# JANUS-Institute/HallThrusterPEM

Measured on AMD Instinct MI355X. Metric: coupled PEM-v0 model evals/sec, higher is better.
Workload: dtype f64

## Files before the change

hallthrusterpem_amd/_lib.py:

```python
import ctypes as C
import importlib.util
import os
import threading
from pathlib import Path

PKG = Path(__file__).resolve().parent
LIB_PATH = PKG / 'libpem_hip.so'

PEM_OK, PEM_ERR_INVALID_ARG, PEM_ERR_HIP, PEM_ERR_NO_DEVICE = 0, 1, 2, 3
NANGLE = 91
FUSED_LATENT_MAX_RANK = 8
FUSED_SYSTEM_MAX_RECORDS = 1024
FUSED_SYSTEM_MAX_RADII = 8
SYS_JION, SYS_VCC, SYS_T, SYS_UION = 0, 1, 2, 3
SWEEP_CATHODE, SWEEP_THRUSTER, SWEEP_PLUME = 0, 1, 2
DE_MAX_POP, DE_MAX_DIM = 1024, 16
DE_BEST1BIN, DE_RAND1BIN = 0, 1
NM_MAX_DIM, NM_STATE_WORDS = 32, 10
POWELL_MAX_DIM, POWELL_STATE_WORDS = 32, 24
POWELL_SCALARS, POWELL_VEC_ROWS = 20, 6
DRAM_MAX_DIM = 32
ENSEMBLE_MAX_DIM, ENSEMBLE_MAX_WALKERS = 32, 1024
SMC_MAX_DIM, SMC_MAX_PARTICLES, SMC_BISECTIONS = 32, 16384, 52
CHAIN_TIME_BLOCK = 4096
# ... 70 lines not shown
    'pem_range_narrow_dev': (C.c_int, [C.c_int, C.c_int, _dp, _dp, _dp, _dp, _dp]),
    'pem_qsel_bins': (C.c_int, [C.c_int, C.c_int, C.POINTER(C.c_int), C.POINTER(C.c_int)]),
    'pem_qsel_minmax_f64_dev': (C.c_int, [_sz, C.c_int, _dp, _sz, _dp, _dp, _dp, _dp]),
    'pem_qsel_hist1_f64_dev': (C.c_int, [_sz, C.c_int, _dp, _sz, _dp, _dp, C.c_int, _dp, _dp]),
    'pem_qsel_decide1_dev': (C.c_int, [C.c_int, C.c_int, _dp, _dp, _dp, C.c_int, _dp, _dp, _dp, _dp, _dp]),
    'pem_qsel_hist2_f64_dev': (C.c_int, [_sz, C.c_int, _dp, _sz, _dp, _dp, C.c_int, _dp, C.c_int, C.c_int, _dp, _dp]),
    'pem_qsel_decide2_dev': (C.c_int, [C.c_int, C.c_int, _dp, _dp, C.c_int, _dp, _dp, _dp, _dp, _dp, _dp, _dp]),
    'pem_qsel_compact_f64_dev': (C.c_int, [_sz, C.c_int, _dp, _sz, _dp, _dp, C.c_int, _dp, _dp, _dp, C.c_int, C.c_int, C.c_uint32, _dp, _dp, _dp]),
    'pem_qsel_select_dev': (C.c_int, [C.c_int, C.c_int, C.c_int, C.c_uint32, _dp, _dp, _dp, _dp, _dp, _dp, _dp]),
    'pem_quantiles_f64_dev': (C.c_int, [_sz, C.c_int, _dp, _sz, C.c_int, _dp, _dp, _dp, _dp, _dp]),
    'pem_quantiles_strided_f64_dev': (C.c_int, [_sz, C.c_int, _dp, _sz, _sz, C.c_int, _dp, _dp, _dp, _dp, _dp]),
    'pem_quantiles_last_path': (C.c_int, []),
    'pem_coupled_mc_stats_f64_dev': (C.c_int, [_sz, C.c_uint64, C.c_uint64, C.c_uint32, _dp, _dp, _dp, C.c_double, C.c_double, _dp, _sz,
                                               _dp, _dp, _dp, _dp, _dp, _dp, _dp, _dp, C.c_int, _dp, _dp, _dp, _dp, _dp, _dp,
                                               C.c_int, C.c_int, C.c_double, _dp, _dp, _dp, _dp]),
    'pem_row_masks_f64_dev': (C.c_int, [_sz, C.c_int, _dp, _sz, _dp, _dp, _dp, _dp, _dp]),
    'pem_campaign_masks_f64_dev': (C.c_int, [_sz, C.c_int, _dp, _dp, C.c_int, C.c_int, C.c_int, C.c_double, _dp, _dp, _sz, _dp, _dp, C.c_int, _dp, _dp,
                                             C.c_int, _dp]),
    'pem_sobol_partial_f64_dev': (C.c_int, [_sz, C.c_int, _sz, _dp, _dp, _dp, _dp, C.c_int, _dp]),
    'pem_coupled_f32_dev': (C.c_int, [_sz, C.c_float, C.c_float, _dp, _sz, _dp, _sz, _dp, _dp]),
    'pem_saltelli_f32_dev': (C.c_int, [_sz, C.c_uint64, C.c_uint64, C.c_uint32, _dp, _dp, _dp, C.c_int, _dp, C.c_float, C.c_float, _dp, _dp, C.c_int, _dp]),
    'pem_saltelli_f64_dev': (C.c_int, [_sz, C.c_uint64, C.c_uint64, C.c_uint32, _dp, _dp, _dp, C.c_int, _dp, C.c_double, C.c_double, _dp, _dp, C.c_int, _dp]),
    'pem_saltelli_qmc_f32_dev': (C.c_int, [_sz, C.c_uint64, C.c_uint64, C.c_uint32, C.c_int, _dp, _dp, _dp, C.c_int, _dp, C.c_float, C.c_float, _dp, _dp,
                                           C.c_int, _dp]),
    'pem_saltelli_qmc_f64_dev': (C.c_int, [_sz, C.c_uint64, C.c_uint64, C.c_uint32, C.c_int, _dp, _dp, _dp, C.c_int, _dp, C.c_double, C.c_double, _dp,
                                           _dp, C.c_int, _dp]),
    'pem_saltelli2_f32_dev': (C.c_int, [_sz, C.c_uint64, C.c_uint64, C.c_uint32, _dp, _dp, _dp, C.c_int, _dp, _dp, C.c_float, C.c_float, _dp, _dp,
                                        C.c_int, _dp]),
    'pem_saltelli2_f64_dev': (C.c_int, [_sz, C.c_uint64, C.c_uint64, C.c_uint32, _dp, _dp, _dp, C.c_int, _dp, _dp, C.c_double, C.c_double, _dp, _dp,
                                        C.c_int, _dp]),
# ... 130 lines not shown
```

hallthrusterpem_amd/build.py:

```python
import os
import shutil
import subprocess
from pathlib import Path

PKG = Path(__file__).resolve().parent
ROOT = PKG.parent
SRCS = [PKG / 'csrc' / 'pem_kernels.hip', PKG / 'csrc' / 'pem_radii.hip', PKG / 'csrc' / 'pem_stages.hip', PKG / 'csrc' / 'pem_host.hip', PKG / 'csrc' / 'pem_campaign.hip', PKG / 'csrc' / 'pem_sampler.hip', PKG / 'csrc' / 'pem_svd.hip', PKG / 'csrc' / 'pem_likelihood.hip', PKG / 'csrc' / 'pem_surrogate.hip', PKG / 'csrc' / 'pem_surrogate_fields.hip', PKG / 'csrc' / 'pem_surrogate_sobol.hip', PKG / 'csrc' / 'pem_fp32.hip', PKG / 'csrc' / 'pem_saltelli.hip', PKG / 'csrc' / 'pem_saltelli2.hip', PKG / 'csrc' / 'pem_latent.hip', PKG / 'csrc' / 'pem_quantile.hip', PKG / 'csrc' / 'pem_masks.hip', PKG / 'csrc' / 'pem_sobol_sweep.hip', PKG / 'csrc' / 'pem_de.hip', PKG / 'csrc' / 'pem_nm.hip', PKG / 'csrc' / 'pem_powell.hip', PKG / 'csrc' / 'pem_dram.hip', PKG / 'csrc' / 'pem_ensemble.hip', PKG / 'csrc' / 'pem_tempering.hip', PKG / 'csrc' / 'pem_smc.hip', PKG / 'csrc' / 'pem_chains.hip', PKG / 'csrc' / 'pem_marginals.hip', PKG / 'csrc' / 'pem_hexbin.hip', PKG / 'csrc' / 'pem_information.hip', PKG / 'csrc' / 'pem_qmc.hip']
LIB = PKG / 'libpem_hip.so'
DEPS = SRCS + sorted((PKG / 'csrc').glob('*.h')) + [ROOT / 'include' / 'pem_hip.h']


def hipcc() -> str:
    exe = shutil.which('hipcc') or '/opt/rocm/bin/hipcc'
    if not Path(exe).exists():
        raise RuntimeError('hipcc not found: libpem_hip.so cannot be built (ROCm toolchain required)')
    return exe


def have_hipcc() -> bool:
    return Path(shutil.which('hipcc') or '/opt/rocm/bin/hipcc').exists()


STAMP = PKG / 'libpem_hip.so.srchash'

# ... 76 lines not shown
```

hallthrusterpem_amd/csrc/pem_qfused.h:

```cpp
#pragma once
#include <hip/hip_runtime.h>

#include <cstdint>

namespace pem {

struct Bracket {
    unsigned long long lo, hi;
    unsigned loh;
    unsigned words;
    unsigned mult;
    unsigned pad;
};

struct Record {
    unsigned long long key;
    unsigned long long col;
};

__device__ __forceinline__ unsigned long long order_key(double x) {
    const unsigned long long b = (unsigned long long)__double_as_longlong(x);
    return (b >> 63) ? ~b : (b | 0x8000000000000000ull);
}
__device__ __forceinline__ unsigned order_key_high(int high_word) {
// ... 24 lines not shown
    size_t ld = 0;
    double *V_cc = nullptr, *I_B0 = nullptr, *T = nullptr, *j_ion = nullptr, *div_angle = nullptr, *T_c = nullptr;
    uint8_t* invalid = nullptr;
};

__attribute__((visibility("hidden"))) int launch_coupled_mc(const McLaunch& a, hipStream_t st);
__attribute__((visibility("hidden"))) int coupled_count_waves(size_t n, int nq, bool store_profile, unsigned* waves);
__attribute__((visibility("hidden"))) int launch_coupled_mc_count(const McLaunch& a, const CountIO& c, bool store_profile, hipStream_t st);

struct FusedProducer {
    virtual ~FusedProducer() {}
    int pm_q25 = -1, pm_q75 = -1;
    double pm_factor = 0.0;
    uint8_t *pm_certain = nullptr, *pm_uncertain = nullptr;
    int pm_done = 0;
    virtual int pilot(size_t rows, double* dst, hipStream_t st) = 0;
    virtual int waves(int nq, unsigned* waves) = 0;
    virtual int count(const CountIO& io, hipStream_t st) = 0;
};
__attribute__((visibility("hidden"))) int quantiles_fused(size_t n, int m, int nq, const uint64_t* rank_prev, const uint64_t* rank_next,
                                                          const double* gamma, double* pilot_rows, FusedProducer& prod, double* out,
                                                          int* fused_ok, hipStream_t st);
struct SidePlan {
    int (*before_full)(void* ctx, hipStream_t st) = nullptr;
    void* ctx = nullptr;
};
__attribute__((visibility("hidden"))) int quantiles_side(size_t n, int m, const double* data, size_t ld, size_t cs, int nq,
                                                         const uint64_t* rank_prev, const uint64_t* rank_next, const double* gamma, double* out,
                                                         hipStream_t st, const SidePlan* plan = nullptr);

// ... 2 lines not shown
```

hallthrusterpem_amd/csrc/pem_quantile.hip:

```cpp
#include <hip/hip_runtime.h>

#include <atomic>
#include <cmath>
#include <cstdint>
#include <cstdlib>
#include <mutex>

#include "pem_common.h"
#include "pem_hip.h"
#include "pem_qfused.h"

namespace {

typedef unsigned long long u64;
constexpr int QBLOCK = 512;
constexpr int QWAVES = QBLOCK / 64;
constexpr int LDS_WORDS = 36864;
constexpr int SORT_CAP = 4096;
constexpr int SORT_DIRECT = 512;
constexpr int MAX_NC = 4;
constexpr int UNROLL = 8;
static_assert(PEM_QUANTILE_MAX_Q == 6, "hist2_kernel / compact_kernel are instantiated for 2, 4, ... 12 ranks per column");

__device__ __forceinline__ u64 key_of(double x) {
// ... 1176 lines not shown
        if (const char* e = getenv("PEM_FUSED_PILOT")) pilot = atoll(e) >= 32 ? atoll(e) : 32;
    }
    if (plan) pilot = 32;
    const bool use_pilot = fused ? true : plan ? (long long)n >= 4 * pilot : (pilot >= 2 && (long long)n * m >= pilot_min && (long long)n >= 4 * pilot);
    if (fused && (long long)n < 4 * pilot) return pem::fail(PEM_ERR_INVALID_ARG, "pem_quantiles: the fused form needs at least %lld rows", 4 * pilot);

    const size_t b_col = sizeof(Column) * m, b_tg = sizeof(Target) * m * nt;
    const size_t b_h1 = sizeof(unsigned) * (size_t)m * bins1, b_h2 = sizeof(unsigned) * (size_t)m * nt * bins2;
    const size_t b_br = sizeof(Bracket) * m * nq, b_bl = sizeof(u64) * m * nq, b_hA = sizeof(unsigned) * (size_t)m * nq * binsA;
    auto up = [](size_t x) { return (x + 255) & ~(size_t)255; };
    const size_t o_tg = up(b_col), o_h1 = o_tg + up(b_tg), o_h2 = o_h1 + up(b_h1), o_tot = o_h2 + up(b_h2);
    unsigned fused_waves = 0;
    if (fused)
        if (int rc = fused->waves(nq, &fused_waves)) return rc;
    const size_t b_rc = sizeof(unsigned) * fused_waves;
    const size_t o_br = o_tot + 256, o_bl = o_br + up(b_br), o_hA = o_bl + up(b_bl), o_rc = o_hA + up(b_hA), o_pm = o_rc + up(b_rc);
    const size_t o_end = o_pm + up(sizeof(uint4) * (size_t)m);
    QWork& work = g_qwork[slot];
    std::lock_guard<std::mutex> lock(work.mu);
    char*& ws_buf = work.ws_buf;
    size_t &ws_cap = work.ws_cap, &cand_cap = work.cand_cap, &rec_cap = work.rec_cap, &part_cap = work.part_cap;
    u64*& cand_buf = work.cand_buf;
    pem::Record*& rec_buf = work.rec_buf;
    unsigned*& part_buf = work.part_buf;
    int& ws_dev = work.ws_dev;
    int dev = 0;
    HIP_TRY(hipGetDevice(&dev));
    if (dev != ws_dev || ws_cap < o_end) {
        if (ws_buf) (void)hipFree(ws_buf);
        if (cand_buf && dev != ws_dev) {
            (void)hipFree(cand_buf);
// ... 18 lines not shown
    }
    char* ws = ws_buf;
    Column* col = reinterpret_cast<Column*>(ws);
    Target* tg = reinterpret_cast<Target*>(ws + o_tg);
    unsigned* hist1 = reinterpret_cast<unsigned*>(ws + o_h1);
    unsigned* hist2 = reinterpret_cast<unsigned*>(ws + o_h2);
    u64* total = reinterpret_cast<u64*>(ws + o_tot);
    int* outside = reinterpret_cast<int*>(total + 1);
    int* incomplete = reinterpret_cast<int*>(total + 2);
    int* any_single = reinterpret_cast<int*>(total + 8);
    int* unfit = reinterpret_cast<int*>(total + 9);
    int* prod_flags = unfit + 1;
    unsigned* rec_count = reinterpret_cast<unsigned*>(ws + o_rc);
    uint4* pm_thr = reinterpret_cast<uint4*>(ws + o_pm);
    int* pm_bad = unfit + 3;
    int* inconsistent = unfit + 4;
    Bracket* br = reinterpret_cast<Bracket*>(ws + o_br);
    u64* below = reinterpret_cast<u64*>(ws + o_bl);
    unsigned* histA = reinterpret_cast<unsigned*>(ws + o_hA);
    auto cleanup = [&](int code) {
        (void)hipStreamSynchronize(st);
        return code;
    };
#define Q_TRY(expr)                                                                                          \
    do {                                                                                                     \
        hipError_t e_ = (expr);                                                                              \
        if (e_ != hipSuccess) return cleanup(pem::fail(PEM_ERR_HIP, "%s: %s", #expr, hipGetErrorString(e_))); \
    } while (0)

    Wanted w{};
    for (int q = 0; q < nq; ++q) {
        w.prev[q] = rank_prev[q];
        w.next[q] = rank_next[q];
        w.gamma[q] = gamma[q];
    }
    const int cblocks = (m + 63) / 64;
    const int nc = m <= 64 ? 1 : (m <= 128 ? 2 : 4);
    const size_t lds1 = (size_t)m * bins1 * 4, lds2 = (size_t)m * nt * bins2 * 4, ldsA = (size_t)m * nq * (binsA + 1) * 4;
    const dim3 blk(QBLOCK);
    auto grid_for = [&](size_t rows) {
        const long long rpw = m <= 64 ? 64 / m : 1, groups = ((long long)rows + rpw - 1) / rpw;
        long long blocks = (groups + (long long)QWAVES * UNROLL - 1) / ((long long)QWAVES * UNROLL);
        if (blocks > 256 * 2) blocks = 256 * 2;
        return dim3((unsigned)blocks);
// ... 101 lines not shown
        PilotEnds ends{};
        const double n1 = n > 1 ? (double)(n - 1) : 1.0, np1 = (double)(rows_p - 1);
        for (int q = 0; q < nq; ++q) {
            const double p_lo = (double)rank_prev[q] / n1, p_hi = (double)rank_next[q] / n1;
            double sig = fused ? 5.0 : 7.0;
            if (fused)
                if (const char* e = getenv("PEM_FUSED_SIGMA")) sig = atof(e) >= 3.0 ? atof(e) : 3.0;
            const double d_lo = sig * sqrt((double)rows_p * p_lo * (1.0 - p_lo)) + 8.0, d_hi = sig * sqrt((double)rows_p * p_hi * (1.0 - p_hi)) + 8.0;
            const double r_lo = floor(p_lo * np1 - d_lo) - 1.0, r_hi = ceil(p_hi * np1 + d_hi) + 1.0;
            ends.open_lo[q] = r_lo < 0.0;
            ends.open_hi[q] = r_hi > np1;
            pw.prev[q] = ends.open_lo[q] ? 0 : (u64)r_lo;
            pw.next[q] = ends.open_hi[q] ? (u64)(rows_p - 1) : (u64)r_hi;
        }
        if (fused) {
            if (int rc = fused->pilot(rows_p, const_cast<double*>(data), st)) return cleanup(rc);
            const bool edges = !(getenv("PEM_FUSED_PILOT_EXACT") && atoi(getenv("PEM_FUSED_PILOT_EXACT")));
            if (int rc = four_passes(rows_p, ld, pw, edges)) return rc;
        } else if (plan) {
            if (int rc = four_passes(rows_p, ld, pw)) return rc;
            if (plan->before_full)
                if (int rc = plan->before_full(plan->ctx, st)) return cleanup(rc);
        } else if (int rc = four_passes(rows_p, ld * (size_t)pilot, pw)) return rc;
        const dim3 grid = grid_for(n);
        Q_TRY(hipMemsetAsync(total, 0, 256, st));
        Q_TRY(hipMemsetAsync(below, 0, o_end - o_bl, st));
        hipLaunchKernelGGL(brackets_kernel, dim3((unsigned)((m * nq + 63) / 64)), dim3(64), 0, st, m, nq, tg, ends, binsA, br, any_single);
        hipLaunchKernelGGL(init_columns_kernel, dim3(cblocks), dim3(64), 0, st, col, tg, m, nq, w);
#define Q_BRHIST_(NC_, NQ_)                                                                                                  \
    Q_LDS((bracket_hist_kernel<NC_, NQ_>));                                                                                  \
    hipLaunchKernelGGL((bracket_hist_kernel<NC_, NQ_>), grid, blk, ldsA, st, (long long)n, m, ld, cs, data, br, any_single, binsA, col, below, histA)
#define Q_BRHIST(NC_) Q_BY_NQ_##NC_(Q_BRHIST_, NC_)
        unsigned rcap = 0;
// ... 69 lines not shown
            hipLaunchKernelGGL(record_reduce_kernel, dim3((unsigned)((cells + 63) / 64)), dim3(256), 0, st, part_buf, cus, cells, histA, rec_count, rcap,
                               fused_waves, rec_sums);
            hipLaunchKernelGGL(record_total_check_kernel, dim3(1), dim3(64), 0, st, rec_sums, inconsistent, prod_flags);
        }
        hipLaunchKernelGGL(decide_bracket_kernel, dim3((unsigned)(m * nt)), dim3(64), 0, st, nt, col, br, below, histA, binsA, tg, outside);
        hipLaunchKernelGGL(layout_kernel, dim3(1), dim3(64 * MAX_NC), 0, st, m, nt, tg, total);
        Q_TRY(hipGetLastError());
        u64 h_tot[2] = {0, 0};
        int h_unfit4[4] = {0, 0, 0, 0};
        Q_TRY(hipMemcpyAsync(h_tot, total, 2 * sizeof(u64), hipMemcpyDeviceToHost, st));
        if (fused) Q_TRY(hipMemcpyAsync(h_unfit4, unfit, sizeof h_unfit4, hipMemcpyDeviceToHost, st));
        Q_TRY(hipStreamSynchronize(st));
        if (fused) fused->pm_done = (pm_launched && h_unfit4[3] == 0) ? 1 : 0;
        if (fused && (h_unfit4[0] || (int)(h_tot[1] & 0xffffffffull) != 0 || h_unfit4[1] || h_unfit4[2])) {
            *fused_ok = 0;
            return cleanup(PEM_OK);
        }
        if ((int)(h_tot[1] & 0xffffffffull) == 0) {
            Q_TRY(grow_candidates(h_tot[0]));
            u64* cand = cand_buf;
#define Q_BRCOMPACT_(NC_, NQ_) \
    hipLaunchKernelGGL((compact_bracket_kernel<NC_, NQ_>), grid, blk, 0, st, (long long)n, m, ld, cs, data, br, tg, cand)
#define Q_BRCOMPACT(NC_) Q_BY_NQ_##NC_(Q_BRCOMPACT_, NC_)
            if (!fused) {
                Q_BY_NC(Q_BRCOMPACT);
            } else {
                int cus = 256;
                Q_TRY(pem::device_cus(&cus));
                unsigned* woff = part_buf + (size_t)cus * m * nq * binsA;
                hipLaunchKernelGGL(record_offsets_kernel, dim3((unsigned)(m * nt)), dim3(64), 0, st, nt, binsA, tg, part_buf, cus, m * nq * binsA, woff);
// ... 626 lines not shown
```

hallthrusterpem_amd/drivers.py:

```python
import functools

import numpy as np

from . import sampling
from .batch import QOI_NAMES, CoupledBatch
from .distributed import shard_bounds

COORDS_STR_ID = '_coords'


MAX_Q, MAX_Q_WIDE = 6, 3


def _linear_ranks(n: int, percentiles):
    return _linear_ranks_cached(int(n), tuple(float(x) for x in np.atleast_1d(np.asarray(percentiles, dtype=np.float64))))


@functools.lru_cache(maxsize=64)
def _linear_ranks_cached(n: int, percentiles: tuple):
    q = np.true_divide(np.asarray(percentiles, dtype=np.float64), np.float64(100))
    if not np.all((q >= 0) & (q <= 1)):
        raise ValueError('Percentiles must be in the range [0, 100]')
    if n == 0:
        raise ValueError('no samples')
# ... 176 lines not shown
            for k in names if k in outputs}


def _stacked_rows(tensors):
    import torch
    t0 = tensors[0]
    if len(tensors) < 2 or any(t.dim() != 1 or not t.is_cuda or t.dtype != torch.float64 or t.numel() != t0.numel() or t.stride(0) != 1
                               or t.untyped_storage().data_ptr() != t0.untyped_storage().data_ptr() for t in tensors):
        return None
    n, step = t0.numel(), tensors[1].storage_offset() - t0.storage_offset()
    if step < n or any(t.storage_offset() != t0.storage_offset() + i * step for i, t in enumerate(tensors)):
        return None
    return torch.as_strided(t0, (n, len(tensors)), (1, step))


def campaign_statistics(outputs: dict, iqr_factor: float = 1.5, percentiles=(5.0, 50.0, 95.0), names=None):
    import torch
    names = [k for k in (outputs if names is None else names) if k in outputs and COORDS_STR_ID not in str(k) and str(k) != 'errors']
    pct = [25.0, 75.0] + [float(x) for x in percentiles]
    q = {}
    scalars = [k for k in names if outputs[k].dim() == 1]
    stacked = _stacked_rows([outputs[k] for k in scalars]) if len(scalars) > 1 else None
    if stacked is not None:
        qs = column_percentiles(stacked, pct)
        q.update({k: qs[:, i] for i, k in enumerate(scalars)})
    for k in names:
        if k not in q:
            q[k] = column_percentiles(outputs[k], pct)
    nan_idx, outlier_idx, bands = {}, {}, {}
    for k in names:
        a, qk = outputs[k].double(), q[k]
        per_sample = int(np.prod(a.shape[1:])) if a.dim() > 1 else 1
        iqr = qk[1] - qk[0]
        lo, hi = qk[0] - iqr_factor * iqr, qk[1] + iqr_factor * iqr
        if a.shape[0] > 0 and per_sample <= ROW_MASKS_MAX_M:
            nan_idx[k], count = _row_masks(a, lo, hi, per_sample)
        else:
            rest = tuple(range(1, a.dim()))
            nan_idx[k] = torch.isnan(a).any(dim=rest) if rest else torch.isnan(a)
            outside = (a < lo) | (a > hi)
            count = outside.sum(dim=rest) if rest else outside.long()
        outlier_idx[k] = count > int(0.75 * per_sample)
        bands[k] = qk[2:]
    return nan_idx, outlier_idx, bands


FUSED_STATS_MIN_N = 4096


def forward_uq_statistics(n: int, seed: int = 0, keep_profile: bool = True, percentiles=(5.0, 50.0, 95.0), iqr_factor: float = 1.5,
                          priors=None, device=None, keep_inputs: bool = False, fused: bool = True):
    import ctypes as C
    import torch
    from . import _lib, constants
    design = sampling.Design(priors=priors, seed=seed)
    batch = CoupledBatch(n, device=device, profile=keep_profile)
    pct = [25.0, 75.0] + [float(x) for x in percentiles]
    answered, premasked, qj, qs, certain, uncertain = False, False, None, None, None, None
    thresh = int(0.75 * _lib.NANGLE)
    nv, cap = len(QOI_NAMES), 65536
    dev = batch.device
    with torch.cuda.device(dev):
        stream = torch.cuda.current_stream(dev)
        n_pad = (n + 3) // 4 * 4
        nan_s = torch.empty((nv + 1, n_pad), dtype=torch.bool, device=dev)[:, :n]
        out_s = torch.empty((nv + 1, n_pad), dtype=torch.bool, device=dev)[:, :n]
        open_rows = torch.empty(cap, dtype=torch.int64, device=dev)
        open_count = torch.zeros(1, dtype=torch.int32, device=dev)
        if fused and n >= FUSED_STATS_MIN_N:
            if len(pct) > MAX_Q:
                raise ValueError(f'the fused campaign takes at most {MAX_Q - 2} percentiles besides the quartiles')
            rp, rn, gm = _linear_ranks(n, pct)
            qj = torch.empty((len(pct), _lib.NANGLE), dtype=torch.float64, device=dev)
            qs = torch.empty((len(pct), nv), dtype=torch.float64, device=dev)
            pilot = None if keep_profile else torch.empty(((n + 31) // 32, _lib.NANGLE), dtype=torch.float64, device=dev)
# ... 33 lines not shown
    q['j_ion'] = qj
    nan_idx, outlier_idx, bands = {}, {}, {}
    dp = lambda t: C.c_void_p(t.data_ptr())
    with torch.cuda.device(dev):
        vars_ = (C.c_void_p * nv)(*[batch.qoi[i].data_ptr() for i in range(nv)])
        _lib.check(_lib.load().pem_campaign_masks_f64_dev(
            n, nv, vars_, dp(qs), qs.stride(0), 0, 1, float(iqr_factor), dp(nan_s), dp(out_s), nan_s.stride(0), dp(certain) if premasked else None,
            dp(uncertain) if premasked else None, thresh, dp(open_rows), dp(open_count), cap, C.c_void_p(torch.cuda.current_stream(dev).cuda_stream)))
    for i, k in enumerate(QOI_NAMES):
        nan_idx[k], outlier_idx[k] = nan_s[i], out_s[i]

    def profile_bounds():
        iqr = qj[1] - qj[0]
        return qj[0] - iqr_factor * iqr, qj[1] + iqr_factor * iqr
    if premasked:
        n_open = int(open_count.item())
        if n_open > cap:
            c, u = certain.to(torch.int32), uncertain.to(torch.int32)
            rows_open = torch.nonzero((c <= thresh) & (c + u > thresh)).flatten()
        else:
            rows_open = open_rows[:n_open]
        outl = out_s[nv]
        if rows_open.numel():
            lo, hi = profile_bounds()
            rows = batch.j_ion[rows_open] if keep_profile else _profile_rows(design, rows_open, device=dev)
            outl[rows_open] = ((rows < lo) | (rows > hi)).sum(dim=1) > thresh
        nan_idx['j_ion'] = nan_s[nv]
        outlier_idx['j_ion'] = outl
    else:
        lo, hi = profile_bounds()
        prof = batch.j_ion if keep_profile else (full.j_ion if full is not None else None)
        if prof is None:
            full = CoupledBatch(n, device=device, profile=True, thruster_qoi=False)
            full.run_mc(design, first_index=0)
            prof = full.j_ion
        nan_idx['j_ion'], count = _row_masks(prof, lo, hi, _lib.NANGLE)
        outlier_idx['j_ion'] = count > thresh
    del full
    for k in q:
        bands[k] = q[k][2:]
    out.update(nan_idx=nan_idx, outlier_idx=outlier_idx, bands=bands, fused=answered, premasked=premasked)
# ... 427 lines not shown
```

include/pem_hip.h:

```cpp
#ifndef PEM_HIP_H
#define PEM_HIP_H

#include <stddef.h>
#include <stdint.h>

#ifdef __cplusplus
extern "C" {
#endif

#define PEM_NANGLE 91

#define PEM_OK 0
#define PEM_ERR_INVALID_ARG 1
#define PEM_ERR_HIP 2
#define PEM_ERR_NO_DEVICE 3

typedef void* pem_stream_t;

const char* pem_version(void);
const char* pem_last_error(void);
int pem_device_count(void);
int pem_init(int device);
int pem_synchronize(pem_stream_t stream);
int pem_set_lanes_per_sample(int lanes);
// ... 208 lines not shown
#define PEM_QUANTILE_MAX_Q_WIDE 3
int pem_quantiles_f64_dev(size_t n, int m, const double* data, size_t ld, int nq, const uint64_t* rank_prev, const uint64_t* rank_next,
                          const double* gamma, double* out, pem_stream_t stream);
int pem_quantiles_strided_f64_dev(size_t n, int m, const double* data, size_t ld, size_t cs, int nq, const uint64_t* rank_prev,
                                  const uint64_t* rank_next, const double* gamma, double* out, pem_stream_t stream);
int pem_quantiles_last_path(void);

#define PEM_MC_STATS_MIN_N 4096
int pem_coupled_mc_stats_f64_dev(size_t n, uint64_t first_index, uint64_t seed, uint32_t stream_id, const int32_t* kind, const double* a,
                                 const double* b, double torr2pa, double radius, double* x_out, size_t ld, double* V_cc, double* I_B0,
                                 double* T, double* j_ion, double* pilot_rows, double* div_angle, double* T_c, uint8_t* invalid, int nq,
                                 const uint64_t* rank_prev, const uint64_t* rank_next, const double* gamma, double* q_out, double* q_scalars,
                                 int* fused_ok, int q25, int q75, double iqr_factor, uint8_t* row_certain, uint8_t* row_uncertain,
                                 int* premask_ok, pem_stream_t stream);

#define PEM_ROW_MASKS_MAX_M 512
int pem_row_masks_f64_dev(size_t n, int m, const double* data, size_t ld, const double* lo, const double* hi, uint8_t* nan_out,
                          int32_t* outside_out, pem_stream_t stream);

int pem_campaign_masks_f64_dev(size_t n, int nvar, const double* const* vars, const double* q, int q_ld, int row25, int row75,
                               double iqr_factor, uint8_t* nan_out,
                               uint8_t* outl_out, size_t mask_ld, const uint8_t* row_certain, const uint8_t* row_uncertain, int thresh,
                               int64_t* open_rows, int32_t* open_count, int cap, pem_stream_t stream);

int pem_key_minmax_f64_dev(size_t n, int m, const double* data, size_t ld, uint64_t* kmin, uint64_t* kmax, int32_t* has_nan,
                           pem_stream_t stream);
int pem_range_hist_f64_dev(size_t n, int m, const double* data, size_t ld, int nr, const uint64_t* klo, const uint64_t* khi,
                           int bins, uint32_t* hist, pem_stream_t stream);
int pem_range_narrow_dev(int n_ranges, int bins, const uint32_t* hist, uint64_t* klo, uint64_t* khi, int64_t* resid,
                         pem_stream_t stream);
// ... 164 lines not shown
```

Before: 7.027 billion.

## Add fused quantile-and-premask counting kernel for stored ion-current profiles

Adds a new HIP counting kernel that reads a stored j_ion profile matrix once. In that one pass it builds the quantile bracket histograms, the candidate records and the per-row certain/uncertain outlier counts. campaign_statistics now sends eligible profile outputs through this fused path instead of a generic column-percentile pass followed by a separate outlier-count pass. Only rows near the threshold are resolved afterwards. This adds a fallback when the fused form declines, plus a new env-tunable wave count.

After: 6.805 billion. -3.2%, worse.

```diff
diff --git a/hallthrusterpem_amd/_lib.py b/hallthrusterpem_amd/_lib.py
--- a/hallthrusterpem_amd/_lib.py
+++ b/hallthrusterpem_amd/_lib.py
@@ -108,6 +108,7 @@
     'pem_coupled_mc_stats_f64_dev': (C.c_int, [_sz, C.c_uint64, C.c_uint64, C.c_uint32, _dp, _dp, _dp, C.c_double, C.c_double, _dp, _sz,
                                                _dp, _dp, _dp, _dp, _dp, _dp, _dp, _dp, C.c_int, _dp, _dp, _dp, _dp, _dp, _dp,
                                                C.c_int, C.c_int, C.c_double, _dp, _dp, _dp, _dp]),
+    'pem_profile_statistics_f64_dev': (C.c_int, [_sz, _dp, C.c_int, _dp, _dp, _dp, _dp, _dp, C.c_int, C.c_int, C.c_double, _dp, _dp, _dp, _dp]),
     'pem_row_masks_f64_dev': (C.c_int, [_sz, C.c_int, _dp, _sz, _dp, _dp, _dp, _dp, _dp]),
     'pem_campaign_masks_f64_dev': (C.c_int, [_sz, C.c_int, _dp, _dp, C.c_int, C.c_int, C.c_int, C.c_double, _dp, _dp, _sz, _dp, _dp, C.c_int, _dp, _dp,
                                              C.c_int, _dp]),
diff --git a/hallthrusterpem_amd/build.py b/hallthrusterpem_amd/build.py
--- a/hallthrusterpem_amd/build.py
+++ b/hallthrusterpem_amd/build.py
@@ -5,7 +5,7 @@
 
 PKG = Path(__file__).resolve().parent
 ROOT = PKG.parent
-SRCS = [PKG / 'csrc' / 'pem_kernels.hip', PKG / 'csrc' / 'pem_radii.hip', PKG / 'csrc' / 'pem_stages.hip', PKG / 'csrc' / 'pem_host.hip', PKG / 'csrc' / 'pem_campaign.hip', PKG / 'csrc' / 'pem_sampler.hip', PKG / 'csrc' / 'pem_svd.hip', PKG / 'csrc' / 'pem_likelihood.hip', PKG / 'csrc' / 'pem_surrogate.hip', PKG / 'csrc' / 'pem_surrogate_fields.hip', PKG / 'csrc' / 'pem_surrogate_sobol.hip', PKG / 'csrc' / 'pem_fp32.hip', PKG / 'csrc' / 'pem_saltelli.hip', PKG / 'csrc' / 'pem_saltelli2.hip', PKG / 'csrc' / 'pem_latent.hip', PKG / 'csrc' / 'pem_quantile.hip', PKG / 'csrc' / 'pem_masks.hip', PKG / 'csrc' / 'pem_sobol_sweep.hip', PKG / 'csrc' / 'pem_de.hip', PKG / 'csrc' / 'pem_nm.hip', PKG / 'csrc' / 'pem_powell.hip', PKG / 'csrc' / 'pem_dram.hip', PKG / 'csrc' / 'pem_ensemble.hip', PKG / 'csrc' / 'pem_tempering.hip', PKG / 'csrc' / 'pem_smc.hip', PKG / 'csrc' / 'pem_chains.hip', PKG / 'csrc' / 'pem_marginals.hip', PKG / 'csrc' / 'pem_hexbin.hip', PKG / 'csrc' / 'pem_information.hip', PKG / 'csrc' / 'pem_qmc.hip']
+SRCS = [PKG / 'csrc' / 'pem_kernels.hip', PKG / 'csrc' / 'pem_radii.hip', PKG / 'csrc' / 'pem_stages.hip', PKG / 'csrc' / 'pem_host.hip', PKG / 'csrc' / 'pem_campaign.hip', PKG / 'csrc' / 'pem_profile_count.hip', PKG / 'csrc' / 'pem_sampler.hip', PKG / 'csrc' / 'pem_svd.hip', PKG / 'csrc' / 'pem_likelihood.hip', PKG / 'csrc' / 'pem_surrogate.hip', PKG / 'csrc' / 'pem_surrogate_fields.hip', PKG / 'csrc' / 'pem_surrogate_sobol.hip', PKG / 'csrc' / 'pem_fp32.hip', PKG / 'csrc' / 'pem_saltelli.hip', PKG / 'csrc' / 'pem_saltelli2.hip', PKG / 'csrc' / 'pem_latent.hip', PKG / 'csrc' / 'pem_quantile.hip', PKG / 'csrc' / 'pem_masks.hip', PKG / 'csrc' / 'pem_sobol_sweep.hip', PKG / 'csrc' / 'pem_de.hip', PKG / 'csrc' / 'pem_nm.hip', PKG / 'csrc' / 'pem_powell.hip', PKG / 'csrc' / 'pem_dram.hip', PKG / 'csrc' / 'pem_ensemble.hip', PKG / 'csrc' / 'pem_tempering.hip', PKG / 'csrc' / 'pem_smc.hip', PKG / 'csrc' / 'pem_chains.hip', PKG / 'csrc' / 'pem_marginals.hip', PKG / 'csrc' / 'pem_hexbin.hip', PKG / 'csrc' / 'pem_information.hip', PKG / 'csrc' / 'pem_qmc.hip']
 LIB = PKG / 'libpem_hip.so'
 DEPS = SRCS + sorted((PKG / 'csrc').glob('*.h')) + [ROOT / 'include' / 'pem_hip.h']
 
diff --git a/hallthrusterpem_amd/csrc/pem_profile_count.hip b/hallthrusterpem_amd/csrc/pem_profile_count.hip
--- /dev/null
+++ b/hallthrusterpem_amd/csrc/pem_profile_count.hip
@@ -0,0 +1,284 @@
+#include "pem_common.h"
+#include "pem_qfused.h"
+
+namespace {
+
+using pem::fail;
+
+constexpr int NANG = PEM_NANGLE;
+constexpr int PC_TILE = 16;
+constexpr int PC_THREADS = 256;
+constexpr int PC_WAVES = 5;
+constexpr int PC_WPB = PC_THREADS / 64;
+static_assert(NANG > 64 && NANG - 64 <= 32, "two slots: columns 0..63, and columns 64..90 two rows per instruction");
+
+template <int NQ>
+struct WaveCounts {
+    unsigned nb[2][NQ];
+    unsigned cnt;
+    unsigned top;
+};
+
+template <int NQ>
+struct SlotTable {
+    uint2 tb[NQ];
+    uint4 th;
+    unsigned long long lanes_on;
+};
+
+template <int NQ, bool PM>
+__device__ __forceinline__ void count_value(int hw, const SlotTable<NQ>& t, unsigned* __restrict__ nb, unsigned& top, unsigned& mine, unsigned bit,
+                                            unsigned long long& certain, unsigned long long& maybe) {
+    const unsigned mag = (unsigned)hw & 0x7fffffffu;
+    top = top > mag ? top : mag;
+    const unsigned kh = pem::order_key_high(hw);
+    unsigned long long in = 0;
+#pragma unroll
+    for (int q = 0; q < NQ; ++q) {
+        unsigned d;
+        nb[q] += __builtin_sub_overflow(kh, t.tb[q].x, &d) ? 1u : 0u;
+        in |= __builtin_amdgcn_uicmp(d, t.tb[q].y, 37 );
+    }
+    mine |= __builtin_amdgcn_inverse_ballot_w64(in) ? bit : 0u;
+    if constexpr (PM) {
+        certain = (__builtin_amdgcn_uicmp(kh, t.th.x, 36 ) | __builtin_amdgcn_uicmp(kh, t.th.w, 34 )) & t.lanes_on;
+        maybe = (__builtin_amdgcn_uicmp(kh, t.th.y, 37 ) | __builtin_amdgcn_uicmp(kh, t.th.z, 35 )) & t.lanes_on & ~certain;
+    }
+}
+
+template <int NQ, bool PM, bool FULL>
+__device__ __forceinline__ void count_tile(const double* __restrict__ p, int rows, long long first, int lane, const uint2* __restrict__ tab,
+                                           const uint4* __restrict__ pmt, pem::Record* __restrict__ rec, unsigned cap,
+                                           uint8_t* __restrict__ row_certain, uint8_t* __restrict__ row_uncertain, WaveCounts<NQ>& w) {
+    unsigned bits = 0;
+    unsigned row_c = 0, row_u = 0;
+    constexpr unsigned long long PART = (1ull << (NANG - 64)) - 1;
+    const int half = FULL ? lane >> 5 : 0, sub = lane & 31;
+    const bool on1 = sub < NANG - 64 && (FULL || lane < 32);
+    const int c1 = sub < NANG - 64 ? 64 + sub : NANG - 1;
+    auto table = [&](int slot) {
+        SlotTable<NQ> t;
+        const int cc = slot == 0 ? lane : c1;
+#pragma unroll
+        for (int q = 0; q < NQ; ++q) t.tb[q] = tab[((slot == 0 || on1) ? cc : NANG) * NQ + q];
+        t.th = make_uint4(0u, 0u, 0u, 0u);
+        if constexpr (PM) t.th = pmt[cc];
+        t.lanes_on = slot == 0 ? ~0ull : (FULL ? (PART | (PART << 32)) : PART);
+        return t;
+    };
+    const double* s0 = p + lane;
+    const double* s1 = p + c1 + half * NANG;
+    unsigned mine0 = 0, mine1 = 0;
+    if constexpr (FULL) {
+#pragma unroll 1
+        for (int g = 0; g < 2; ++g) {
+            int h0[8], h1[4];
+#pragma unroll
+            for (int u = 0; u < 8; ++u) h0[u] = __double2hiint(s0[(8 * g + u) * NANG]);
+#pragma unroll
+            for (int u = 0; u < 4; ++u) h1[u] = __double2hiint(s1[2 * (4 * g + u) * NANG]);
+            {
+                const SlotTable<NQ> t = table(0);
+#pragma unroll
+                for (int tt = 0; tt < 2; ++tt) {
+                    const int turn = 2 * g + tt;
+                    unsigned pc = 0, pu = 0;
+#pragma unroll
+                    for (int u = 0; u < 4; ++u) {
+                        unsigned long long certain = 0, maybe = 0;
+                        count_value<NQ, PM>(h0[4 * tt + u], t, w.nb[0], w.top, mine0, 1u << (4 * turn + u), certain, maybe);
+                        if constexpr (PM) {
+                            pc |= (unsigned)__popcll(certain) << (8 * u);
+                            pu |= (unsigned)__popcll(maybe) << (8 * u);
+                        }
+                    }
+                    if constexpr (PM) {
+                        row_c += lane == turn ? pc : 0u;
+                        row_u += lane == turn ? pu : 0u;
+                    }
+                    __builtin_amdgcn_sched_barrier(0);
+                }
+            }
+            {
+                const SlotTable<NQ> t = table(1);
+                const unsigned bit0 = 1u << (16 + half);
+#pragma unroll
+                for (int tt = 0; tt < 2; ++tt) {
+                    const int turn = 2 * g + tt;
+                    unsigned pc = 0, pu = 0;
+#pragma unroll
+                    for (int u = 0; u < 2; ++u) {
+                        unsigned long long certain = 0, maybe = 0;
+                        count_value<NQ, PM>(h1[2 * tt + u], t, w.nb[1], w.top, mine1, bit0 << (4 * turn + 2 * u), certain, maybe);
+                        if constexpr (PM) {
+                            pc |= ((unsigned)__popc((unsigned)certain) << (16 * u)) | ((unsigned)__popc((unsigned)(certain >> 32)) << (16 * u + 8));
+                            pu |= ((unsigned)__popc((unsigned)maybe) << (16 * u)) | ((unsigned)__popc((unsigned)(maybe >> 32)) << (16 * u + 8));
+                        }
+                        __builtin_amdgcn_sched_barrier(0);
+                    }
+                    if constexpr (PM) {
+                        row_c += lane == turn ? pc : 0u;
+                        row_u += lane == turn ? pu : 0u;
+                    }
+                }
+            }
+        }
+    } else {
+        const SlotTable<NQ> t0 = table(0), t1 = table(1);
+#pragma unroll 1
+        for (int r = 0; r < rows; ++r) {
+            unsigned long long c0 = 0, m0 = 0, c1m = 0, m1 = 0;
+            const int a = __double2hiint(s0[r * NANG]), b = __double2hiint(s1[r * NANG]);
+            count_value<NQ, PM>(a, t0, w.nb[0], w.top, mine0, 1u << r, c0, m0);
+            count_value<NQ, PM>(b, t1, w.nb[1], w.top, mine1, 1u << (16 + r), c1m, m1);
+            if constexpr (PM) {
+                row_c += lane == r ? (unsigned)(__popcll(c0) + __popcll(c1m)) : 0u;
+                row_u += lane == r ? (unsigned)(__popcll(m0) + __popcll(m1)) : 0u;
+            }
+        }
+    }
+    bits = mine0 | (on1 ? mine1 : 0u);
+    if constexpr (PM) {
+        if constexpr (FULL) {
+            if (lane < PC_TILE / 4) {
+                reinterpret_cast<unsigned*>(row_certain + first)[lane] = row_c;
+                reinterpret_cast<unsigned*>(row_uncertain + first)[lane] = row_u;
+            }
+        } else if (lane < rows) {
+            row_certain[first + lane] = (uint8_t)row_c;
+            row_uncertain[first + lane] = (uint8_t)row_u;
+        }
+    }
+    unsigned cnt = w.cnt;
+    while (__ballot(bits != 0)) {
+        const bool has0 = bits != 0;
+        const int b0 = has0 ? __builtin_ctz(bits) : 0;
+        bits &= bits - 1;
+        const bool has1 = bits != 0;
+        const int b1 = has1 ? __builtin_ctz(bits) : 0;
+        bits &= bits - 1;
+        const int col0 = (b0 >> 4) ? 64 + (lane & 31) : lane, col1 = (b1 >> 4) ? 64 + (lane & 31) : lane;
+        const double x0 = p[has0 ? (b0 & 15) * NANG + col0 : 0], x1 = p[has1 ? (b1 & 15) * NANG + col1 : 0];
+        const unsigned long long e0 = __ballot(has0), e1 = __ballot(has1);
+        const unsigned at0 = cnt + __builtin_amdgcn_mbcnt_hi((unsigned)(e0 >> 32), __builtin_amdgcn_mbcnt_lo((unsigned)e0, 0u));
+        const unsigned n0 = (unsigned)__popcll(e0);
+        const unsigned at1 = cnt + n0 + __builtin_amdgcn_mbcnt_hi((unsigned)(e1 >> 32), __builtin_amdgcn_mbcnt_lo((unsigned)e1, 0u));
+        if (has0 && at0 < cap) *reinterpret_cast<ulonglong2*>(rec + at0) = make_ulonglong2(pem::order_key(x0), (unsigned long long)col0);
+        if (has1 && at1 < cap) *reinterpret_cast<ulonglong2*>(rec + at1) = make_ulonglong2(pem::order_key(x1), (unsigned long long)col1);
+        cnt += n0 + (unsigned)__popcll(e1);
+    }
+    w.cnt = cnt;
+}
+
+template <int NQ, bool PM>
+__global__ __launch_bounds__(PC_THREADS) __attribute__((amdgpu_waves_per_eu(PC_WAVES))) void profile_count_kernel(
+    const double* __restrict__ data, long long n, pem::CountIO io) {
+    __shared__ uint2 tab[(NANG + 1) * NQ];
+    __shared__ uint4 pmt[PM ? NANG : 1];
+    __shared__ unsigned below[NQ * NANG];
+    const int tid = threadIdx.x, lane = tid & 63, wave = tid >> 6;
+    for (int i = tid; i < NANG * NQ; i += PC_THREADS) {
+        const int c = i / NQ, q = i - c * NQ;
+        tab[i] = q < io.nq ? make_uint2(io.br[c * io.nq + q].loh, io.br[c * io.nq + q].words) : make_uint2(0xffffffffu, 0u);
+        below[i] = 0;
+    }
+    if (tid < NQ) tab[NANG * NQ + tid] = make_uint2(0u, 0u);
+    if constexpr (PM)
+        for (int i = tid; i < NANG; i += PC_THREADS) pmt[i] = io.premask[i];
+    __syncthreads();
+
+    WaveCounts<NQ> w;
+#pragma unroll
+    for (int q = 0; q < NQ; ++q) w.nb[0][q] = w.nb[1][q] = 0;
+    w.cnt = 0;
+    w.top = 0;
+    const long long me = (long long)blockIdx.x * PC_WPB + wave, nwaves = (long long)gridDim.x * PC_WPB;
+    const long long nfull = n / PC_TILE, ntiles = (n + PC_TILE - 1) / PC_TILE;
+    pem::Record* rec = io.rec + (size_t)me * io.cap;
+    for (long long t = me; t < nfull; t += nwaves)
+        count_tile<NQ, PM, true>(data + t * PC_TILE * NANG, PC_TILE, t * PC_TILE, lane, tab, pmt, rec, io.cap, io.row_certain, io.row_uncertain, w);
+    if (nfull < ntiles && (nfull % nwaves) == me)
+        count_tile<NQ, PM, false>(data + nfull * PC_TILE * NANG, (int)(n - nfull * PC_TILE), nfull * PC_TILE, lane, tab, pmt, rec, io.cap,
+                                  io.row_certain, io.row_uncertain, w);
+
+#pragma unroll
+    for (int q = 0; q < NQ; ++q) {
+        if (w.nb[0][q]) atomicAdd(&below[q * NANG + lane], w.nb[0][q]);
+        if ((lane & 31) < NANG - 64 && w.nb[1][q]) atomicAdd(&below[q * NANG + 64 + (lane & 31)], w.nb[1][q]);
+    }
+    if (__ballot(w.top >= 0x7ff00000u) && lane == 0) atomicOr(io.flags + 1, 1);
+    if (lane == 0) {
+        io.rec_count[me] = w.cnt;
+        if (w.cnt > io.cap) atomicOr(io.flags, 1);
+    }
+    __syncthreads();
+    for (int i = tid; i < NQ * NANG; i += PC_THREADS) {
+        const int q = i / NANG, c = i - q * NANG;
+        if (below[i] && q < io.nq) atomicAdd(&io.below[c * io.nq + q], (unsigned long long)below[i]);
+    }
+}
+
+int count_waves(unsigned* waves) {
+    int cus = 0;
+    HIP_TRY(pem::device_cus(&cus));
+    long long per_cu = 4 * PC_WAVES;
+    if (const char* e = getenv("PEM_PROFILE_COUNT_WAVES_PER_CU")) per_cu = atoll(e);
+    per_cu = per_cu < PC_WPB ? PC_WPB : (per_cu > 32 ? 32 : per_cu / PC_WPB * PC_WPB);
+    *waves = (unsigned)(cus * per_cu);
+    return PEM_OK;
+}
+
+struct StoredProducer : pem::FusedProducer {
+    const double* data = nullptr;
+    size_t n = 0;
+    int pilot(size_t, double*, hipStream_t) override { return PEM_OK; }
+    int waves(int, unsigned* w) override { return count_waves(w); }
+    int count(const pem::CountIO& io, hipStream_t st) override {
+        if (io.nq < 1 || io.nq > 6 || !io.br || !io.below || !io.rec || !io.rec_count || !io.flags || io.cap == 0)
+            return fail(PEM_ERR_INVALID_ARG, "pem_profile_statistics: incomplete arguments of the counting launch");
+        unsigned wv = 0;
+        PEM_TRY(count_waves(&wv));
+        const dim3 grid(wv / PC_WPB), blk(PC_THREADS);
+        const bool pm = io.premask && io.row_certain && io.row_uncertain && io.nq <= 5;
+        if (pm)
+            hipLaunchKernelGGL((profile_count_kernel<5, true>), grid, blk, 0, st, data, (long long)n, io);
+        else if (io.nq <= 5)
+            hipLaunchKernelGGL((profile_count_kernel<5, false>), grid, blk, 0, st, data, (long long)n, io);
+        else
+            hipLaunchKernelGGL((profile_count_kernel<6, false>), grid, blk, 0, st, data, (long long)n, io);
+        HIP_TRY(hipGetLastError());
+        return PEM_OK;
+    }
+};
+
+}
+
+extern "C" int pem_profile_statistics_f64_dev(size_t n, const double* j_ion, int nq, const uint64_t* rank_prev, const uint64_t* rank_next,
+                                              const double* gamma, double* q_out, int* fused_ok, int q25, int q75, double iqr_factor,
+                                              uint8_t* row_certain, uint8_t* row_uncertain, int* premask_ok, pem_stream_t stream) {
+    if (!j_ion || !rank_prev || !rank_next || !gamma || !q_out || !fused_ok) return fail(PEM_ERR_INVALID_ARG, "pem_profile_statistics: NULL array");
+    if (!pem::aligned16(j_ion)) return fail(PEM_ERR_INVALID_ARG, "pem_profile_statistics: j_ion must be 16-byte aligned");
+    if (nq < 1 || nq > PEM_QUANTILE_MAX_Q) return fail(PEM_ERR_INVALID_ARG, "pem_profile_statistics: 1 <= nq <= %d", PEM_QUANTILE_MAX_Q);
+    if (n < PEM_MC_STATS_MIN_N || n >= (1ull << 31))
+        return fail(PEM_ERR_INVALID_ARG, "pem_profile_statistics: %d <= n < 2^31 samples", PEM_MC_STATS_MIN_N);
+    if ((reinterpret_cast<uintptr_t>(row_certain) | reinterpret_cast<uintptr_t>(row_uncertain)) & 3u)
+        return fail(PEM_ERR_INVALID_ARG, "pem_profile_statistics: row_certain / row_uncertain must be 4-byte aligned");
+    if (int rc = pem::check_device()) return rc;
+    StoredProducer prod;
+    prod.data = j_ion;
+    prod.n = n;
+    prod.pilot_strided = true;
+    if (row_certain && row_uncertain && premask_ok) {
+        prod.pm_q25 = q25;
+        prod.pm_q75 = q75;
+        prod.pm_factor = iqr_factor;
+        prod.pm_certain = row_certain;
+        prod.pm_uncertain = row_uncertain;
+    }
+    if (premask_ok) *premask_ok = 0;
+    *fused_ok = 0;
+    PEM_TRY(pem::quantiles_fused(n, PEM_NANGLE, nq, rank_prev, rank_next, gamma, const_cast<double*>(j_ion), prod, q_out, fused_ok,
+                                 static_cast<hipStream_t>(stream)));
+    if (premask_ok) *premask_ok = (*fused_ok && prod.pm_done) ? 1 : 0;
+    return PEM_OK;
+}
diff --git a/hallthrusterpem_amd/csrc/pem_qfused.h b/hallthrusterpem_amd/csrc/pem_qfused.h
--- a/hallthrusterpem_amd/csrc/pem_qfused.h
+++ b/hallthrusterpem_amd/csrc/pem_qfused.h
@@ -62,6 +62,7 @@
     double pm_factor = 0.0;
     uint8_t *pm_certain = nullptr, *pm_uncertain = nullptr;
     int pm_done = 0;
+    bool pilot_strided = false;
     virtual int pilot(size_t rows, double* dst, hipStream_t st) = 0;
     virtual int waves(int nq, unsigned* waves) = 0;
     virtual int count(const CountIO& io, hipStream_t st) = 0;
diff --git a/hallthrusterpem_amd/csrc/pem_quantile.hip b/hallthrusterpem_amd/csrc/pem_quantile.hip
--- a/hallthrusterpem_amd/csrc/pem_quantile.hip
+++ b/hallthrusterpem_amd/csrc/pem_quantile.hip
@@ -1214,7 +1214,7 @@
     if (fused)
         if (int rc = fused->waves(nq, &fused_waves)) return rc;
     const size_t b_rc = sizeof(unsigned) * fused_waves;
-    const size_t o_br = o_tot + 256, o_bl = o_br + up(b_br), o_hA = o_bl + up(b_bl), o_rc = o_hA + up(b_hA), o_pm = o_rc + up(b_rc);
+    const size_t o_br = o_tot + 512, o_bl = o_br + up(b_br), o_hA = o_bl + up(b_bl), o_rc = o_hA + up(b_hA), o_pm = o_rc + up(b_rc);
     const size_t o_end = o_pm + up(sizeof(uint4) * (size_t)m);
     QWork& work = g_qwork[slot];
     std::lock_guard<std::mutex> lock(work.mu);
@@ -1263,7 +1263,7 @@
     unsigned* rec_count = reinterpret_cast<unsigned*>(ws + o_rc);
     uint4* pm_thr = reinterpret_cast<uint4*>(ws + o_pm);
     int* pm_bad = unfit + 3;
-    int* inconsistent = unfit + 4;
+    int* inconsistent = reinterpret_cast<int*>(ws + o_tot + 256);
     Bracket* br = reinterpret_cast<Bracket*>(ws + o_br);
     u64* below = reinterpret_cast<u64*>(ws + o_bl);
     unsigned* histA = reinterpret_cast<unsigned*>(ws + o_hA);
@@ -1277,6 +1277,7 @@
         if (e_ != hipSuccess) return cleanup(pem::fail(PEM_ERR_HIP, "%s: %s", #expr, hipGetErrorString(e_))); \
     } while (0)
 
+    Q_TRY(hipMemsetAsync(inconsistent, 0, 256, st));
     Wanted w{};
     for (int q = 0; q < nq; ++q) {
         w.prev[q] = rank_prev[q];
@@ -1408,9 +1409,10 @@
             pw.next[q] = ends.open_hi[q] ? (u64)(rows_p - 1) : (u64)r_hi;
         }
         if (fused) {
-            if (int rc = fused->pilot(rows_p, const_cast<double*>(data), st)) return cleanup(rc);
+            if (!fused->pilot_strided)
+                if (int rc = fused->pilot(rows_p, const_cast<double*>(data), st)) return cleanup(rc);
             const bool edges = !(getenv("PEM_FUSED_PILOT_EXACT") && atoi(getenv("PEM_FUSED_PILOT_EXACT")));
-            if (int rc = four_passes(rows_p, ld, pw, edges)) return rc;
+            if (int rc = four_passes(rows_p, fused->pilot_strided ? ld * (size_t)pilot : ld, pw, edges)) return rc;
         } else if (plan) {
             if (int rc = four_passes(rows_p, ld, pw)) return rc;
             if (plan->before_full)
@@ -1510,6 +1512,9 @@
         if (fused) fused->pm_done = (pm_launched && h_unfit4[3] == 0) ? 1 : 0;
         if (fused && (h_unfit4[0] || (int)(h_tot[1] & 0xffffffffull) != 0 || h_unfit4[1] || h_unfit4[2])) {
             *fused_ok = 0;
+            if (getenv("PEM_QUANTILE_TRACE"))
+                fprintf(stderr, "pem_quantiles (fused form) declined: unfit brackets %d, rank outside its bracket %d, record overflow %d, non-finite %d (waves %u, cap %u)\n",
+                        h_unfit4[0], (int)(h_tot[1] & 0xffffffffull), h_unfit4[1], h_unfit4[2], fused_waves, rcap);
             return cleanup(PEM_OK);
         }
         if ((int)(h_tot[1] & 0xffffffffull) == 0) {
diff --git a/hallthrusterpem_amd/drivers.py b/hallthrusterpem_amd/drivers.py
--- a/hallthrusterpem_amd/drivers.py
+++ b/hallthrusterpem_amd/drivers.py
@@ -214,6 +214,75 @@
     return torch.as_strided(t0, (n, len(tensors)), (1, step))
 
 
+FUSED_STATS_MIN_N = 4096
+_PREMASK_OPEN_CAP = 65536
+
+
+def _settle_premask(outl, certain, uncertain, open_rows, open_count, cap: int, thresh: int, bounds, rows_of):
+    import torch
+    n_open = int(open_count.item())
+    if n_open > cap:
+        c, u = certain.to(torch.int32), uncertain.to(torch.int32)
+        rows_open = torch.nonzero((c <= thresh) & (c + u > thresh)).flatten()
+    else:
+        rows_open = open_rows[:n_open]
+    if rows_open.numel():
+        lo, hi = bounds()
+        rows = rows_of(rows_open)
+        outl[rows_open] = ((rows < lo) | (rows > hi)).sum(dim=1) > thresh
+    return outl
+
+
+_STORED_PATHS = {}
+
+
+def campaign_statistics_paths():
+    return dict(_STORED_PATHS)
+
+
+def _takes_stored_profile(a, nq: int) -> bool:
+    import torch
+    from . import _lib
+    return (a.is_cuda and a.dtype == torch.float64 and a.dim() == 2 and a.shape[1] == _lib.NANGLE and a.is_contiguous() and
+            FUSED_STATS_MIN_N <= a.shape[0] < 2 ** 31 and nq <= MAX_Q and a.data_ptr() % 16 == 0)
+
+
+def _stored_profile_statistics(a, pct, iqr_factor: float):
+    import ctypes as C
+    import torch
+    from . import _lib
+    n, dev = int(a.shape[0]), a.device
+    thresh, cap = int(0.75 * _lib.NANGLE), _PREMASK_OPEN_CAP
+    rp, rn, gm = _linear_ranks(n, pct)
+    ptr = lambda arr: C.c_void_p(arr.ctypes.data)
+    dp = lambda t: C.c_void_p(t.data_ptr())
+    with torch.cuda.device(dev):
+        stream = C.c_void_p(torch.cuda.current_stream(dev).cuda_stream)
+        qj = torch.empty((len(pct), _lib.NANGLE), dtype=torch.float64, device=dev)
+        n_pad = (n + 3) // 4 * 4
+        certain = torch.empty(n_pad, dtype=torch.uint8, device=dev)
+        uncertain = torch.empty(n_pad, dtype=torch.uint8, device=dev)
+        nan_s = torch.empty((1, n_pad), dtype=torch.bool, device=dev)[:, :n]
+        out_s = torch.empty((1, n_pad), dtype=torch.bool, device=dev)[:, :n]
+        open_rows = torch.empty(cap, dtype=torch.int64, device=dev)
+        open_count = torch.zeros(1, dtype=torch.int32, device=dev)
+        ok, pm_ok = C.c_int(0), C.c_int(0)
+        _lib.check(_lib.load().pem_profile_statistics_f64_dev(n, dp(a), len(pct), ptr(rp), ptr(rn), ptr(gm), dp(qj), C.byref(ok), 0, 1, float(iqr_factor),
+                                                              dp(certain), dp(uncertain), C.byref(pm_ok), stream))
+        if not ok.value:
+            return None
+        if not pm_ok.value:
+            return qj, None, None
+        _lib.check(_lib.load().pem_campaign_masks_f64_dev(n, 0, None, None, 0, 0, 1, float(iqr_factor), dp(nan_s), dp(out_s), nan_s.stride(0), dp(certain),
+                                                          dp(uncertain), thresh, dp(open_rows), dp(open_count), cap, stream))
+
+    def bounds():
+        iqr = qj[1] - qj[0]
+        return qj[0] - iqr_factor * iqr, qj[1] + iqr_factor * iqr
+    outl = _settle_premask(out_s[0], certain, uncertain, open_rows, open_count, cap, thresh, bounds, lambda rows: a[rows])
+    return qj, nan_s[0], outl
+
+
 def campaign_statistics(outputs: dict, iqr_factor: float = 1.5, percentiles=(5.0, 50.0, 95.0), names=None):
     import torch
     names = [k for k in (outputs if names is None else names) if k in outputs and COORDS_STR_ID not in str(k) and str(k) != 'errors']
@@ -224,12 +293,27 @@
     if stacked is not None:
         qs = column_percentiles(stacked, pct)
         q.update({k: qs[:, i] for i, k in enumerate(scalars)})
+    nan_idx, outlier_idx, bands, counted = {}, {}, {}, {}
+    _STORED_PATHS.clear()
     for k in names:
-        if k not in q:
+        if k in q:
+            _STORED_PATHS[k] = 'passes'
+            continue
+        res = _stored_profile_statistics(outputs[k], pct, iqr_factor) if _takes_stored_profile(outputs[k], len(pct)) else None
+        if res is None:
+            _STORED_PATHS[k] = 'declined' if _takes_stored_profile(outputs[k], len(pct)) else 'passes'
             q[k] = column_percentiles(outputs[k], pct)
-    nan_idx, outlier_idx, bands = {}, {}, {}
+            continue
+        q[k] = res[0]
+        _STORED_PATHS[k] = 'counted' if res[1] is not None else 'counted, masks by a pass'
+        if res[1] is not None:
+            counted[k] = res[1:]
     for k in names:
         a, qk = outputs[k].double(), q[k]
+        bands[k] = qk[2:]
+        if k in counted:
+            nan_idx[k], outlier_idx[k] = counted[k]
+            continue
         per_sample = int(np.prod(a.shape[1:])) if a.dim() > 1 else 1
         iqr = qk[1] - qk[0]
         lo, hi = qk[0] - iqr_factor * iqr, qk[1] + iqr_factor * iqr
@@ -241,11 +325,7 @@
             outside = (a < lo) | (a > hi)
             count = outside.sum(dim=rest) if rest else outside.long()
         outlier_idx[k] = count > int(0.75 * per_sample)
-        bands[k] = qk[2:]
     return nan_idx, outlier_idx, bands
-
-
-FUSED_STATS_MIN_N = 4096
 
 
 def forward_uq_statistics(n: int, seed: int = 0, keep_profile: bool = True, percentiles=(5.0, 50.0, 95.0), iqr_factor: float = 1.5,
@@ -258,7 +338,7 @@
     pct = [25.0, 75.0] + [float(x) for x in percentiles]
     answered, premasked, qj, qs, certain, uncertain = False, False, None, None, None, None
     thresh = int(0.75 * _lib.NANGLE)
-    nv, cap = len(QOI_NAMES), 65536
+    nv, cap = len(QOI_NAMES), _PREMASK_OPEN_CAP
     dev = batch.device
     with torch.cuda.device(dev):
         stream = torch.cuda.current_stream(dev)
@@ -322,17 +402,8 @@
         iqr = qj[1] - qj[0]
         return qj[0] - iqr_factor * iqr, qj[1] + iqr_factor * iqr
     if premasked:
-        n_open = int(open_count.item())
-        if n_open > cap:
-            c, u = certain.to(torch.int32), uncertain.to(torch.int32)
-            rows_open = torch.nonzero((c <= thresh) & (c + u > thresh)).flatten()
-        else:
-            rows_open = open_rows[:n_open]
-        outl = out_s[nv]
-        if rows_open.numel():
-            lo, hi = profile_bounds()
-            rows = batch.j_ion[rows_open] if keep_profile else _profile_rows(design, rows_open, device=dev)
-            outl[rows_open] = ((rows < lo) | (rows > hi)).sum(dim=1) > thresh
+        outl = _settle_premask(out_s[nv], certain, uncertain, open_rows, open_count, cap, thresh, profile_bounds,
+                               (lambda rows: batch.j_ion[rows]) if keep_profile else (lambda rows: _profile_rows(design, rows, device=dev)))
         nan_idx['j_ion'] = nan_s[nv]
         outlier_idx['j_ion'] = outl
     else:
diff --git a/include/pem_hip.h b/include/pem_hip.h
--- a/include/pem_hip.h
+++ b/include/pem_hip.h
@@ -246,6 +246,10 @@
                                  int* fused_ok, int q25, int q75, double iqr_factor, uint8_t* row_certain, uint8_t* row_uncertain,
                                  int* premask_ok, pem_stream_t stream);
 
+int pem_profile_statistics_f64_dev(size_t n, const double* j_ion, int nq, const uint64_t* rank_prev, const uint64_t* rank_next,
+                                   const double* gamma, double* q_out, int* fused_ok, int q25, int q75, double iqr_factor,
+                                   uint8_t* row_certain, uint8_t* row_uncertain, int* premask_ok, pem_stream_t stream);
+
 #define PEM_ROW_MASKS_MAX_M 512
 int pem_row_masks_f64_dev(size_t n, int m, const double* data, size_t ld, const double* lo, const double* hi, uint8_t* nan_out,
                           int32_t* outside_out, pem_stream_t stream);
```
